# nrontsis/PILCO

Hardware: AMD Instinct MI355X
Metric: moment-matching rollouts/sec (N=1000,D=10,E=10,H=40) (higher is better)
Workload: dtype f64

## Files before the change

pilco_amd/csrc/prep_device.h:

```cpp
#pragma once
#include "glue_device.h"
#include "pair_device.h"

namespace pilco {

constexpr int PREP_TAB_DOUBLES = FEXP_TN + 8;
__host__ __device__ constexpr size_t prep_region_doubles(int DT) {
    const size_t stage = 256 * (size_t)(DT + 1),
                 ops = mm_kp(DT) <= 16 ? (size_t)mm_kp(DT) * (64 + 256) + 256 + (DT <= 14 ? 16 * 64 + 256 + 8 * 64 : 0) : 0;
    const size_t pair_blk = (size_t)4 * DT + 2 * (size_t)DT * DT + 4 + (stage > ops ? stage : ops);
    const size_t mean_blk = (size_t)2 * DT + 2 * (size_t)DT * DT + 4 + 9 * (size_t)(DT + 1) + 2 * (size_t)DT + 512 * (size_t)(DT + 2);
    return pair_blk > mean_blk ? pair_blk : mean_blk;
}

template <int DT>
__device__ __forceinline__ void prep_wt_constants(const MMModel& md, const MMWork& wk, int pl, double* sm) {
    const int R = wt_rows_per_pair(wk), t = threadIdx.x;
    if (wt_rows_dealt(wk) && t < R && pl * R + t < md.E * md.D) {
        const double l = md.ls[pl * R + t];
        sm[3 * DT + 2 * DT * DT + 4 + t] = 1.0 / (l * l);
    }
}

template <int DT, bool FUSED, int NTHR, bool PRE = false>
__device__ __forceinline__ void prep_mean_block(const MMModel& md, const MMWork& wk, int al, int chm, double* sm,
                                                const double* jm, const double* js,
                                                const double la_t, const double var_a) {
    const int D = md.D, npad = md.npad;
    const int t = threadIdx.x, lane = t & 63;
    const int w = __builtin_amdgcn_readfirstlane(t >> 6);
    const bool act = (NTHR == 512) || t < 512;
    const int a = al * wk.nranks + wk.rank;
    double* s_m = sm;
    double* s_ia = s_m + DT;
    double* s_s = s_ia + DT;
    double* s_T = s_s + DT * DT;
    double* s_sc = s_T + DT * DT;
    double* red = s_sc + 4;
    double* colbuf = red + 9 * (DT + 1);
    double* zst = colbuf + 2 * DT;
    double* bst = zst + 512 * (DT + 1);
    constexpr int LDZ = DT | 1;
    if constexpr (!PRE) {
        if (t < DT) {
            s_m[t] = (t < D) ? (FUSED ? jm[t] : wk.in_m[t]) : 0.0;
            s_ia[t] = (t < D) ? 1.0 / la_t : 0.0;
        }
        for (int e = t; e < D * D; e += 512) s_s[e] = FUSED ? js[e] : wk.in_s[e];
        for (int e = t; e < DT * DT; e += 512) s_T[e] = 0.0;
        __syncthreads();
    }
    const bool dbgm = (t == 0 && al == 0 && chm == 0);
    DBG_STAMP(wk, 40, dbgm);
    const int rpc = npad >> __builtin_ctz(wk.NCHM);
    const int i_begin = chm * rpc, i_end = i_begin + rpc;
    if (w == 0) {
        double col[DT];
        const int c = lane;
        const bool in_s = c < D;
        const double ic = in_s ? s_ia[c] : 0.0;
        double sv[DT], ir[DT];
#pragma unroll
        for (int r = 0; r < DT; ++r) {
            sv[r] = s_s[(in_s && r < D) ? r * D + c : 0];
            ir[r] = s_ia[r];
        }
#pragma unroll
        for (int r = 0; r < DT; ++r) {
            const double sval = (in_s && r < D) ? sv[r] : 0.0;
            col[r] = c < DT ? fma(sval, ir[r] * ic, (r == c) ? 1.0 : 0.0) : ((c < 2 * DT && c - DT == r) ? 1.0 : 0.0);
        }
        __builtin_amdgcn_s_setprio(3);
        const double detB = gj_wave<DT>(col, colbuf, lane);
        __builtin_amdgcn_s_setprio(0);
        if (c >= DT && c < DT + D) {
            const int cc = c - DT;
#pragma unroll
            for (int r = 0; r < DT; ++r)
                if (r < D) s_T[r * DT + cc] = col[r] * s_ia[r] * s_ia[cc];
        }
        if (lane == 0) s_sc[1] = var_a * fast_rsqrt(detB);
    } else if (act) {
        const int idx = (w - 1) * 64 + lane;
        constexpr int NB = (512 * DT + 447) / 448;
        double sv[NB], bv[2];
#pragma unroll
        for (int k = 0; k < NB; ++k) {
            const int e = idx + 448 * k, d = e >> 9, i = i_begin + (e & 511);
            sv[k] = (e < 512 * D && i < md.n && i < i_end) ? md.Pt[(long)d * npad + i] : 0.0;
        }
#pragma unroll
        for (int k = 0; k < 2; ++k) {
            const int r = idx + 448 * k;
            bv[k] = (r < 512 && i_begin + r < i_end) ? md.beta[mm_beta_row(md, a) * npad + i_begin + r] : 0.0;
        }
#pragma unroll
        for (int k = 0; k < NB; ++k) {
            const int e = idx + 448 * k, d = e >> 9, r = e & 511, i = i_begin + r;
            if (e < 512 * D) zst[r * LDZ + d] = (i < md.n && i < i_end) ? sv[k] - s_m[d] : 0.0;
        }
#pragma unroll
        for (int k = 0; k < 2; ++k)
            if (idx + 448 * k < 512) bst[idx + 448 * k] = bv[k];
    }
    __syncthreads();
    DBG_STAMP(wk, 41, dbgm);
    double g = 0.0;
    double h[DT];
#pragma unroll
    for (int d = 0; d < DT; ++d) h[d] = 0.0;
    for (int r0 = 0; r0 < rpc; r0 += 512) {
        if (r0 > 0) {
            __syncthreads();
            for (int e = t; act && e < 512 * D; e += 512) {
                const int d = e >> 9, r = e & 511;
                const int i = i_begin + r0 + r;
                zst[r * LDZ + d] = (i < md.n && i < i_end) ? md.Pt[(long)d * npad + i] - s_m[d] : 0.0;
            }
            if (act) bst[t] = (i_begin + r0 + t < i_end) ? md.beta[mm_beta_row(md, a) * npad + i_begin + r0 + t] : 0.0;
            __syncthreads();
        }
        if (act && i_begin + r0 + t < i_end) {
            double zeta[DT];
#pragma unroll
            for (int d = 0; d < DT; ++d) zeta[d] = (d < D) ? zst[t * LDZ + d] : 0.0;
            double hq = 0.0;
#pragma unroll
            for (int c = 0; c < DT; ++c) {
                double inner = 0.5 * s_T[c * DT + c] * zeta[c];
#pragma unroll
                for (int r = c + 1; r < DT; ++r) inner = fma(s_T[c * DT + r], zeta[r], inner);
                hq = fma(zeta[c], inner, hq);
            }
            const double lb = exp(-hq) * bst[t];
            g += lb;
#pragma unroll
            for (int d = 0; d < DT; ++d) h[d] = fma(zeta[d], lb, h[d]);
        }
    }
    DBG_STAMP(wk, 42, dbgm);
    double* hs = red + 8 * (DT + 1);
    __syncthreads();
    if (act) {
        zst[t] = g;
#pragma unroll
        for (int d = 0; d < DT; ++d)
            if (d < D) zst[(1 + d) * 512 + t] = h[d];
    }
    __syncthreads();
    for (int k = w; act && k < 1 + D; k += 8) {
        double acc = zst[k * 512 + lane];
#pragma unroll
        for (int j = 1; j < 8; ++j) acc += zst[k * 512 + 64 * j + lane];
        acc = wave_sum_lane63(acc);
        if (lane == 63) hs[k] = acc;
    }
    DBG_STAMP(wk, 43, dbgm);
    __syncthreads();
    if (t < 1 + D) {
        double v;
        if (t == 0) {
            v = s_sc[1] * hs[0];
        } else {
            double acc = 0.0;
            _Pragma("unroll 8") for (int k = 0; k < D; ++k) acc = fma(s_T[(t - 1) * DT + k], hs[1 + k], acc);
            v = s_sc[1] * acc;
        }
        store_wt(&wk.mean_part[((long)al * wk.NCHM + chm) * (1 + D) + t], v);
    }
    DBG_STAMP(wk, 44, dbgm);
}

template <int DT>
__device__ __forceinline__ void small_sweep(const MMModel& md, const MMWork& wk, int pl, int item, int i_begin, int c_begin, int ncols, const double* Al, const double* Bl,
                                            const double* vl, const double* Zl, double* bbl, double* csl, double* tail, bool act) {
    constexpr int KC = mm_kp(DT) / 4;
    constexpr bool VSEP = mm_vsep(DT);
    const int D = md.D, npad = md.npad, t = threadIdx.x, lane = t & 63, lr = lane >> 4, lc = lane & 15;
    const int w = __builtin_amdgcn_readfirstlane(t >> 6);
    const double* tab = tail;
    int a, b;
    local_pair_ab(wk, md.E, pl, a, b);
    const bool diag = (a == b);
    const double* beta_a = md.beta + mm_beta_row(md, a) * npad;
    const double* beta_b = md.beta + mm_beta_row(md, b) * npad;
    const double* iKa = (diag && md.iK) ? md.iK + mm_ik_blk(md, a) * npad * npad : nullptr;
    if (act)
        for (int e = t; e < 256; e += 512) bbl[e] = e < npad ? beta_b[e] : 0.0;
    for (int e = t; e < 8 * 64; e += 512) csl[e] = 0.0;
    __syncthreads();
    const int rg = w >> 2, cq = w & 3;
    const int i0l = 32 * rg, i0 = i_begin + i0l;
    const int cpw = ncols / 4, jb = c_begin + cpw * cq, je = jb + cpw;
    double rf[2][KC], brow[2];
#pragma unroll
    for (int rt = 0; rt < 2; ++rt) {
        brow[rt] = beta_a[i0 + 16 * rt + lc];
#pragma unroll
        for (int c = 0; c < KC; ++c) rf[rt][c] = Al[(4 * c + lr) * 64 + i0l + 16 * rt + lc];
    }
    const __amdgpu_buffer_rsrc_t rIK = buf_rsrc_uniform(iKa ? iKa : beta_a);
    unsigned ik_off[2][4];
#pragma unroll
    for (int r = 0; r < 4; ++r)
#pragma unroll
        for (int rt = 0; rt < 2; ++rt) ik_off[rt][r] = ((unsigned)(lr + 4 * r) * (unsigned)npad + (unsigned)(i0 + 16 * rt + lc)) * 8u;
    const int dsel = lc <= D ? lc : D;
    d4 acc[2] = {d4{0.0, 0.0, 0.0, 0.0}, d4{0.0, 0.0, 0.0, 0.0}};
    double* myslice = csl + w * 64;
    auto sweep = [&](auto mode_c) {
        constexpr int MODE = decltype(mode_c)::value;
        double ikv[4][2][4];
        if (MODE == 1) {
#pragma unroll
            for (int sidx = 0; sidx < 4; ++sidx) {
                const int j0 = jb + 16 * sidx;
#pragma unroll
                for (int rt = 0; rt < 2; ++rt)
#pragma unroll
                    for (int r = 0; r < 4; ++r)
                        ikv[sidx][rt][r] = (j0 < je && j0 >= i0) ? buf_ld(rIK, ik_off[rt][r], (unsigned)j0 * (unsigned)npad * 8u) : 0.0;
            }
        }
#pragma unroll
        for (int sidx = 0; sidx < 4; ++sidx) {
            const int j0 = jb + 16 * sidx;
            if (j0 >= je) break;
            if (MODE != 0 && j0 < i0) continue;
            double cf[KC], a2[4], bcol[4], vj[4];
#pragma unroll
            for (int c = 0; c < KC; ++c) cf[c] = Bl[(4 * c + lr) * 256 + j0 + lc];
#pragma unroll
            for (int r = 0; r < 4; ++r) {
                bcol[r] = bbl[j0 + lr + 4 * r];
                vj[r] = VSEP ? vl[j0 + lr + 4 * r] : 0.0;
                a2[r] = Bl[dsel * 256 + j0 + 4 * r + lr];
            }
            double csum[4] = {0.0, 0.0, 0.0, 0.0};
#pragma unroll
            for (int rt = 0; rt < 2; ++rt) {
                const int it = i0 + 16 * rt;
                const double om = j0 > it ? 2.0 : (j0 == it ? 1.0 : 0.0);
                d4 e = {0.0, 0.0, 0.0, 0.0};
#pragma unroll
                for (int c = 0; c < KC; ++c) {
                    e = __builtin_amdgcn_mfma_f64_16x16x4f64(cf[c], rf[rt][c], e, 0, 0, 0);
                    if (c == 0) MFMA_PIN(e, cf[0], rf[rt][0]);
                }
                MFMA_RESULT_FENCE(e);
                double wl[4];
#pragma unroll
                for (int r = 0; r < 4; ++r) {
                    const double l = fexp(VSEP ? e[r] + vj[r] : e[r], tab);
                    if (MODE == 0) {
                        wl[r] = bcol[r] * l;
                        csum[r] = fma(brow[rt], l, csum[r]);
                    } else {
                        double wgt = brow[rt] * bcol[r];
                        if (MODE == 1) wgt -= ikv[sidx][rt][r];
                        wl[r] = (wgt * om) * l;
                        csum[r] += wl[r];
                    }
                }
#pragma unroll
                for (int r = 0; r < 4; ++r) {
                    acc[rt] = __builtin_amdgcn_mfma_f64_16x16x4f64(wl[r], a2[r], acc[rt], 0, 0, 0);
                    MFMA_PIN(acc[rt], wl[r], a2[r]);
                }
            }
#pragma unroll
            for (int r = 0; r < 4; ++r) {
                double v = csum[r];
                v = dpp_add<0x111, 0xf>(v);
                v = dpp_add<0x112, 0xf>(v);
                v = dpp_add<0x114, 0xf>(v);
                v = dpp_add<0x118, 0xf>(v);
                if (lc == 15) myslice[j0 - jb + lr + 4 * r] = v;
            }
        }
    };
    if (act) {
        if (!diag) sweep(std::integral_constant<int, 0>{});
        else if (iKa) sweep(std::integral_constant<int, 1>{});
        else sweep(std::integral_constant<int, 2>{});
    }
    d4 G = {0.0, 0.0, 0.0, 0.0}, Gc = {0.0, 0.0, 0.0, 0.0};
    const int rlane = (lane & 48) | (D & 15);
    if (act) {
#pragma unroll
        for (int rt = 0; rt < 2; ++rt)
#pragma unroll
            for (int r = 0; r < 4; ++r) {
                const int il = i0l + 16 * rt + 4 * r + lr, i = i_begin + il;
                const bool valid = i < md.n;
                const double zt = (valid && lc <= D) ? Zl[lc * 64 + il] : 0.0;
                const double bs = !valid ? 0.0 : (diag ? 1.0 : beta_a[i]);
                const double ri = __shfl(acc[rt][r], rlane);
                const double x = acc[rt][r];
                const double mp = bs == 0.0 ? 0.0 : (lc < D ? fma(0.5 * ri, zt, x) : x);
                const double za = zt * bs;
                G = __builtin_amdgcn_mfma_f64_16x16x4f64(za, mp, G, 0, 0, 0);
                MFMA_PIN(G, za, mp);
            }
    }
    __syncthreads();
    if (act) {
        const int cw8 = ncols / 8;
#pragma unroll
        for (int k = 0; k < 8; ++k) {
            if (4 * k >= cw8) break;
            const int jl = cw8 * w + 4 * k + lr, j = c_begin + jl;
            const int q = jl / cpw;
            double cj = 0.0, wt = 0.0;
            if (j < md.n) {
                const int jj = jl - cpw * q;
                cj = (csl[q * 64 + jj] + csl[(4 + q) * 64 + jj]) * (diag ? 1.0 : bbl[j]);
                wt = lc <= D ? Bl[lc * 256 + j] : 0.0;
            }
            const double ca = cj * wt;
            Gc = __builtin_amdgcn_mfma_f64_16x16x4f64(ca, wt, Gc, 0, 0, 0);
            MFMA_PIN(Gc, ca, wt);
        }
    }
    __syncthreads();
    double* red = const_cast<double*>(Bl);
    double* gout = wk.sw_gpart + ((long)pl * wk.NT + item) * 512;
    const int tN = ((D & 15) >> 2) * 64 + (D & 3) * 16 + (D & 15);
    for (int blk = 0; blk < 2; ++blk) {
        if (blk) __syncthreads();
        d4 v4 = blk ? Gc : G;
        MFMA_RESULT_FENCE(v4);
        if (act) {
#pragma unroll
            for (int r = 0; r < 4; ++r) red[w * 256 + r * 64 + lane] = v4[r];
        }
        __syncthreads();
        if (t < 256) {
            double v = red[t];
#pragma unroll
            for (int k = 1; k < 8; ++k) v += red[k * 256 + t];
            gout[blk * 256 + t] = v;
            if (blk == 0 && t == tN) {
                double* o = wk.pair_part + ((long)pl * wk.NT + item) * 2;
                store_wt(o, v);
                store_wt(o + 1, 0.0);
            }
        }
    }
}

template <int DT, bool FUSED, int NTHR, bool FPAIR = false, bool PRE = false>
__device__ __forceinline__ void prep_work(const MMModel& md, const MMWork& wk, const PrepReward& pr, const GlueArgs& g, const GlueLds& L,
                                          double* sm_all, int glue_doubles, int bx, int by, int gx, int gy, int pair_a, int pair_b, double pre_la, double pre_lb,
                                          double pre_var) {
    double* sm = sm_all + (FUSED ? glue_doubles : 0);
    const bool state_in = FUSED && (g.flags & GF_RBF_PRE);
    const double* jm = sm_all + (state_in ? 0 : L.o_js - L.nm);
    const double* js = sm_all + (state_in ? L.o_sx : L.o_js);
    if (bx >= wk.PL) {
        const int idx = (bx - wk.PL) * gy + by;
        const int nmean = wk.EL * wk.NCHM;
        const int slot = 64 + 2 * (by * gx + bx);
        if (wk.dbg && threadIdx.x == 0 && slot < 958) wk.dbg[slot] = wall_clock64();
        if (idx < nmean) {
            prep_mean_block<DT, FUSED, NTHR, PRE>(md, wk, idx >> __builtin_ctz(wk.NCHM), idx & (wk.NCHM - 1), sm, jm, js, pre_la, pre_var);
            if (wk.dbg && threadIdx.x == 0 && slot < 958) wk.dbg[slot + 1] = wall_clock64();
            return;
        }
        if (idx != nmean || pr.n <= 0) return;
        const int E = pr.E, t = threadIdx.x;
        double* mx = sm;
        double* sx = mx + E;
        double* ws = sx + E * E;
        if (FUSED) {
            if (t < E) mx[t] = L.mx[t];
            for (int e = t; e < E * E; e += blockDim.x) sx[e] = L.sx[e];
        } else {
            if (t < E) mx[t] = pr.m_x[t];
            for (int e = t; e < E * E; e += blockDim.x) sx[e] = pr.s_x[e];
        }
        __syncthreads();
        double mu, var;
        reward_eval(pr.n, pr.rw, E, mx, sx, ws, false, mu, var);
        if (t == 0) pr.reward[0] += mu;
        if (wk.dbg && t == 0 && slot < 958) wk.dbg[slot + 1] = wall_clock64();
        return;
    }
    const int D = md.D, npad = md.npad;
    double* s_m = sm;
    double* s_ia2 = s_m + DT;
    double* s_ib2 = s_ia2 + DT;
    double* s_s = s_ib2 + DT;
    double* s_Q = s_s + DT * DT;
    double* s_sc = s_Q + DT * DT;
    double* colbuf = s_sc + 4;
    double* zst = colbuf + DT;
    const int t = threadIdx.x, lane = t & 63;
    const int w = __builtin_amdgcn_readfirstlane(t >> 6);
    const bool act = (NTHR == 512) || t < 512;
    const int grp = t >> 8, tl = t & 255;
    const int pl = bx, ch = by & (wk.NCH - 1), cs = by >> __builtin_ctz(wk.NCH);
    const bool dbg0 = (t == 0 && pl == 0 && ch == 0);
    DBG_STAMP(wk, 0, dbg0);
    if (wk.dbg && t == 0) wk.dbg[64 + 2 * (by * gx + bx)] = wall_clock64();
    if constexpr (!PRE) {
        if (t < DT) {
            double la = 1.0, lb = 1.0, mm = 0.0;
            if (t < D) {
                mm = FUSED ? jm[t] : wk.in_m[t];
                la = pre_la;
                lb = pre_lb;
            }
            s_m[t] = mm;
            s_ia2[t] = (t < D) ? 1.0 / (la * la) : 0.0;
            s_ib2[t] = (t < D) ? 1.0 / (lb * lb) : 0.0;
        }
        prep_wt_constants<DT>(md, wk, pl, sm);
        for (int e = t; e < D * D; e += 512) s_s[e] = FUSED ? js[e] : wk.in_s[e];
        for (int e = t; e < DT * DT; e += 512) s_Q[e] = 0.0;
        __syncthreads();
    }
    DBG_STAMP(wk, 1, dbg0);
    const int rpc = npad >> __builtin_ctz(wk.NCH);
    const int i_begin = ch * rpc, i_end = i_begin + rpc;
    const int side = grp;
    constexpr int LDZ = DT | 1;
    const bool fpair = FPAIR && wk.fuse_pair;
    const bool fplds = fpair && mm_kp(DT) <= 16 && rpc == 64;
    const int ncsg = (fplds && wk.NCS > 1) ? wk.NCS : 1, ncols = npad >> __builtin_ctz(ncsg), c_begin = cs * ncols, c_end = c_begin + ncols;
    double* Al = zst;
    double* Bl = Al + mm_kp(DT) * 64;
    double* vl = Bl + mm_kp(DT) * 256;
    const bool fsweep = fplds && DT <= 14 && wk.fuse_pair == 2;
    double* Zl = vl + 256;
    double* bbl = Zl + 16 * 64;
    double* csl = bbl + 256;
    const int st_begin = fpair ? 0 : i_begin, st_end = fpair ? npad : i_end;
    if (w != 0 && act) {
        const int idx = (w - 1) * 64 + lane;
        for (int e = idx; e < 256 * D; e += 448) {
            const int d = e >> 8, r = e & 255;
            const int i = st_begin + r;
            zst[r * LDZ + d] = (i < md.n && i < st_end) ? md.Pt[(long)d * npad + i] - s_m[d] : 0.0;
        }
        DBG_STAMP(wk, 7, t == 64 && pl == 0 && ch == 0);
    }
    const double logvar = pre_var;
    if (MM_ABL(wk, 2)) {
        if (t == 0) s_sc[0] = 1.0;
    } else if (w == 0) {
        double col[DT];
        const int c = lane;
        const int cc = c < DT ? c : c - DT;
        const bool in_s = cc < D && c < 2 * DT;
        const double lam = (c < DT && c < D) ? s_ia2[c] + s_ib2[c] : 0.0;
        double sv[DT];
#pragma unroll
        for (int r = 0; r < DT; ++r) sv[r] = s_s[(in_s && r < D) ? r * D + cc : 0];
#pragma unroll
        for (int r = 0; r < DT; ++r) {
            const double sval = (in_s && r < D) ? sv[r] : 0.0;
            col[r] = c < DT ? fma(sval, lam, (r == c) ? 1.0 : 0.0) : sval;
        }
        DBG_STAMP(wk, 5, dbg0);
        __builtin_amdgcn_s_setprio(3);
        const double det = gj_wave<DT>(col, colbuf, lane);
        __builtin_amdgcn_s_setprio(0);
        DBG_STAMP(wk, 6, dbg0);
        if (c >= DT && c < DT + D) {
#pragma unroll
            for (int r = 0; r < DT; ++r)
                if (r < D) s_Q[r * DT + (c - DT)] = 0.5 * col[r];
        }
        if (lane == 0) {
            s_sc[0] = fast_rsqrt(det);
            if (by == 0) store_wt(&wk.pair_isdet[pl], s_sc[0]);
        }
    }
    __syncthreads();
    DBG_STAMP(wk, 2, dbg0);
    const int KP = wk.KP;
    const int pa_ = pair_a, pb_ = pair_b;
    double* At = wk.At + (long)pl * KP * npad;
    double* Wb = wk.Wt + (long)pair_col_block(wk, pl, pb_) * KP * npad;
    double* vrow = wk.vcol + (long)pl * npad;
    const bool wt_dealt = wt_rows_dealt(wk);
    const bool wt_writer = !wt_dealt && pair_writes_wt(wk, md.E, pa_, pb_);
    const int wt_R = wt_rows_per_pair(wk);
    auto row = [&](const int i, const bool valid, const double (&zeta)[DT]) {
        const double* il2 = side ? s_ib2 : s_ia2;
        double x[DT], y[DT];
        double kk = logvar;
#pragma unroll
        for (int d = 0; d < DT; ++d) {
            x[d] = zeta[d] * il2[d];
            kk = fma(-0.5 * zeta[d], x[d], kk);
            y[d] = 0.0;
        }
        DBG_STAMP_ROW(wk, 34, dbg0);
#pragma unroll
        for (int c = 0; c < DT; ++c) {
            double qrow[DT];
#pragma unroll
            for (int r = 0; r < DT; ++r) qrow[r] = s_Q[c * DT + r];
#pragma unroll
            for (int r = 0; r < DT; ++r) y[r] = fma(qrow[r], x[c], y[r]);
            if ((c & 1) == 1) __builtin_amdgcn_sched_barrier(0);
        }
        double quad = 0.0;
#pragma unroll
        for (int r = 0; r < DT; ++r) quad = fma(x[r], y[r], quad);
        DBG_STAMP_ROW(wk, 35, dbg0);
        const double uv = valid ? (kk + quad) : 0.0;
        const double one = valid ? 1.0 : 0.0;
        if (fplds) {
            if (side == 0) {
                const int il = i - i_begin;
#pragma unroll
                for (int r = 0; r < DT; ++r)
                    if (r < D) Al[r * 64 + il] = 2.0 * y[r];
                Al[D * 64 + il] = uv;
                if (!wk.vsep) Al[(D + 1) * 64 + il] = one;
                for (int k = D + 2; k < KP; ++k) Al[k * 64 + il] = 0.0;
                if (fsweep) {
#pragma unroll
                    for (int r = 0; r < DT; ++r)
                        if (r < D) Zl[r * 64 + il] = x[r];
                    Zl[D * 64 + il] = one;
                }
            } else {
#pragma unroll
                for (int r = 0; r < DT; ++r)
                    if (r < D) Bl[r * 256 + i] = x[r];
                Bl[D * 256 + i] = one;
                if (wk.vsep) vl[i] = uv;
                else Bl[(D + 1) * 256 + i] = uv;
                for (int k = D + 2; k < KP; ++k) Bl[k * 256 + i] = 0.0;
            }
        } else if (side == 0) {
#pragma unroll
            for (int r = 0; r < DT; ++r)
                if (r < D) store_wt(&At[(long)r * npad + i], 2.0 * y[r]);
            store_wt(&At[(long)D * npad + i], uv);
        } else {
            if (wt_writer) {
#pragma unroll
                for (int r = 0; r < DT; ++r)
                    if (r < D) store_wt(&Wb[(long)r * npad + i], x[r]);
            }
            store_wt(&vrow[i], uv);
            if (wt_dealt) {
                for (int q = 0; q < wt_R; ++q) {
                    const int rr = pl * wt_R + q;
                    if (rr >= md.E * D) break;
                    int dd;
                    const int bb = idiv_s(rr, D, dd);
                    store_wt(&wk.Wt[((long)bb * KP + dd) * npad + i], zst[(i - st_begin) * LDZ + dd] * colbuf[q]);
                }
            }
        }
    };
    if (fplds) {
        const int r_begin = side ? c_begin : i_begin, r_end = side ? c_end : i_end;
        const bool has = act && r_begin + tl < r_end;
        const int i = r_begin + tl;
        double zeta[DT];
#pragma unroll
        for (int d = 0; d < DT; ++d) zeta[d] = (has && d < D) ? zst[(i - st_begin) * LDZ + d] : 0.0;
        __syncthreads();
        if (has) row(i, i < md.n, zeta);
    } else if (!MM_ABL(wk, 4) && act) {
        const int r_begin = (fpair && side) ? 0 : i_begin, r_end = (fpair && side) ? npad : i_end;
        if (r_begin + tl < r_end) {
            const int i = r_begin + tl;
            double zeta[DT];
#pragma unroll
            for (int d = 0; d < DT; ++d) zeta[d] = (d < D) ? zst[(i - st_begin) * LDZ + d] : 0.0;
            row(i, i < md.n, zeta);
        }
        for (int i = i_begin + tl + 256; i < i_end; i += 256) {
            const bool valid = i < md.n;
            double zeta[DT];
#pragma unroll
            for (int d = 0; d < DT; ++d) zeta[d] = (d < D && valid) ? md.Pt[(long)d * npad + i] - s_m[d] : 0.0;
            row(i, valid, zeta);
        }
    }
    DBG_STAMP(wk, 3, dbg0);
    if (fsweep) {
        small_sweep<DT>(md, wk, pl, by, i_begin, c_begin, ncols, Al, Bl, vl, Zl, bbl, csl, sm + prep_region_doubles(DT), act);
    } else if (fpair) {
        constexpr int KCP = mm_kp(DT) / 4;
        constexpr bool VSP = mm_vsep(DT);
        const double* tab = sm + prep_region_doubles(DT);
        double* wred = sm + prep_region_doubles(DT) + FEXP_TN;
        __syncthreads();
        int a, b;
        local_pair_ab(wk, md.E, pl, a, b);
        const bool diag = (a == b) && (md.iK != nullptr);
        const int nrg = rpc / (16 * PAIR_RT), ncs = max(1, 8 / nrg);
        double val = 0.0;
        if (act && w < nrg * ncs) {
            const int rg = w / ncs, cq = w - rg * ncs, ct = ncols / 16;
            const int i0 = i_begin + 16 * PAIR_RT * rg, jb = c_begin + 16 * (ct * cq / ncs), je = c_begin + 16 * (ct * (cq + 1) / ncs);
            const double* beta_a = md.beta + mm_beta_row(md, a) * npad;
            const double* beta_b = md.beta + mm_beta_row(md, b) * npad;
            const double* iKa = diag ? md.iK + mm_ik_blk(md, a) * npad * npad : nullptr;
            const PairOps po = pair_ops(wk, D, npad, pl, pair_col_block(wk, pl, b));
            if (fplds && mm_kp(DT) <= 16) {
                if (diag) val = pair_wave<KCP, true, VSP, true, true>(po, Al, Bl, vl, beta_a, beta_b, iKa, tab, npad, i0, jb, je, lane, 64, 256, i0 - i_begin);
                else val = pair_wave<KCP, false, VSP, true, true>(po, Al, Bl, vl, beta_a, beta_b, nullptr, tab, npad, i0, jb, je, lane, 64, 256, i0 - i_begin);
            } else if (diag) {
                val = pair_wave<KCP, true, VSP, true>(po, nullptr, nullptr, nullptr, beta_a, beta_b, iKa, tab, npad, i0, jb, je, lane);
            } else {
                val = pair_wave<KCP, false, VSP, true>(po, nullptr, nullptr, nullptr, beta_a, beta_b, nullptr, tab, npad, i0, jb, je, lane);
            }
            for (int off = 32; off > 0; off >>= 1) val += __shfl_down(val, off);
        }
        if (act && lane == 0) wred[w] = val;
        __syncthreads();
        if (t == 0) {
            double* out = wk.pair_part + ((long)pl * wk.NT + by) * 2;
            store_wt(out, ((wred[0] + wred[1]) + (wred[2] + wred[3])) + ((wred[4] + wred[5]) + (wred[6] + wred[7])));
            store_wt(out + 1, 0.0);
        }
    }
    DBG_STAMP(wk, 4, dbg0);
    if (wk.dbg && t == 0) wk.dbg[65 + 2 * (by * gx + bx)] = wall_clock64();
}

}
```

Measured before the change: 416.4.

## Compute per-row quadratic forms with f64 MFMA tiles instead of scalar rows

Measured after the change: 416.9 (median of 6 runs). About the same (+0.1%).

```diff
diff --git a/pilco_amd/csrc/prep_device.h b/pilco_amd/csrc/prep_device.h
--- a/pilco_amd/csrc/prep_device.h
+++ b/pilco_amd/csrc/prep_device.h
@@ -570,20 +570,119 @@
         __syncthreads();
         if (has) row(i, i < md.n, zeta);
     } else if (!MM_ABL(wk, 4) && act) {
+        constexpr int KC = (DT + 3) / 4, MT = (DT + 15) / 16;
+        const int lr = lane >> 4, lc = lane & 15, ws = tl >> 6;
+        const double* il2 = side ? s_ib2 : s_ia2;
+        double qa[MT][KC], il[KC];
+#pragma unroll
+        for (int c = 0; c < KC; ++c) {
+            const int k = 4 * c + lr;
+            il[c] = k < DT ? il2[k] : 0.0;
+#pragma unroll
+            for (int mt = 0; mt < MT; ++mt) qa[mt][c] = (k < DT && 16 * mt + lc < DT) ? s_Q[(16 * mt + lc) * DT + k] : 0.0;
+        }
+        constexpr int TG = DT <= 16 ? 4 : 1;
+        auto tiles = [&](const int (&i)[TG], const bool (&in_r)[TG], const double (&zeta)[TG][KC]) {
+            double x[TG][KC], part[TG];
+            d4 y[TG][MT];
+#pragma unroll
+            for (int g = 0; g < TG; ++g) {
+                part[g] = 0.0;
+#pragma unroll
+                for (int c = 0; c < KC; ++c) {
+                    x[g][c] = zeta[g][c] * il[c];
+                    part[g] = fma(-0.5 * zeta[g][c], x[g][c], part[g]);
+                }
+            }
+#pragma unroll
+            for (int g = 0; g < TG; ++g)
+#pragma unroll
+                for (int mt = 0; mt < MT; ++mt) {
+                    y[g][mt] = d4{0.0, 0.0, 0.0, 0.0};
+#pragma unroll
+                    for (int c = 0; c < KC; ++c) {
+                        y[g][mt] = __builtin_amdgcn_mfma_f64_16x16x4f64(qa[mt][c], x[g][c], y[g][mt], 0, 0, 0);
+                        if (c == 0) MFMA_PIN(y[g][mt], qa[mt][0], x[g][0]);
+                    }
+                }
+#pragma unroll
+            for (int g = 0; g < TG; ++g)
+#pragma unroll
+                for (int mt = 0; mt < MT; ++mt) {
+                    MFMA_RESULT_FENCE(y[g][mt]);
+#pragma unroll
+                    for (int r = 0; r < 4; ++r)
+                        if (4 * mt + r < KC) part[g] = fma(x[g][4 * mt + r], y[g][mt][r], part[g]);
+                }
+#pragma unroll
+            for (int g = 0; g < TG; ++g) part[g] += __shfl_xor(part[g], 16);
+#pragma unroll
+            for (int g = 0; g < TG; ++g) part[g] += __shfl_xor(part[g], 32);
+#pragma unroll
+            for (int g = 0; g < TG; ++g) {
+                if (!in_r[g]) continue;
+                const double uv = i[g] < md.n ? logvar + part[g] : 0.0;
+                if (side == 0) {
+#pragma unroll
+                    for (int mt = 0; mt < MT; ++mt)
+#pragma unroll
+                        for (int r = 0; r < 4; ++r) {
+                            const int m = 16 * mt + lr + 4 * r;
+                            if (m < D) store_wt(&At[(long)m * npad + i[g]], 2.0 * y[g][mt][r]);
+                        }
+                    if (lr == 0) store_wt(&At[(long)D * npad + i[g]], uv);
+                } else {
+                    if (wt_writer) {
+#pragma unroll
+                        for (int c = 0; c < KC; ++c)
+                            if (4 * c + lr < D) store_wt(&Wb[(long)(4 * c + lr) * npad + i[g]], x[g][c]);
+                    }
+                    if (lr == 0) store_wt(&vrow[i[g]], uv);
+                    if (wt_dealt) {
+                        for (int q = lr; q < wt_R; q += 4) {
+                            const int rr = pl * wt_R + q;
+                            if (rr >= md.E * D) break;
+                            int dd;
+                            const int bb = idiv_s(rr, D, dd);
+                            store_wt(&wk.Wt[((long)bb * KP + dd) * npad + i[g]], zst[(i[g] - st_begin) * LDZ + dd] * colbuf[q]);
+                        }
+                    }
+                }
+            }
+        };
         const int r_begin = (fpair && side) ? 0 : i_begin, r_end = (fpair && side) ? npad : i_end;
-        if (r_begin + tl < r_end) {
-            const int i = r_begin + tl;
-            double zeta[DT];
-#pragma unroll
-            for (int d = 0; d < DT; ++d) zeta[d] = (d < D) ? zst[(i - st_begin) * LDZ + d] : 0.0;
-            row(i, i < md.n, zeta);
-        }
-        for (int i = i_begin + tl + 256; i < i_end; i += 256) {
-            const bool valid = i < md.n;
-            double zeta[DT];
-#pragma unroll
-            for (int d = 0; d < DT; ++d) zeta[d] = (d < D && valid) ? md.Pt[(long)d * npad + i] - s_m[d] : 0.0;
-            row(i, valid, zeta);
+#pragma unroll
+        for (int k0 = 0; k0 < 4; k0 += TG) {
+            if (r_begin + 64 * ws + 16 * k0 >= r_end) break;
+            int i[TG];
+            bool in_r[TG];
+            double zeta[TG][KC];
+#pragma unroll
+            for (int g = 0; g < TG; ++g) {
+                i[g] = r_begin + 64 * ws + 16 * (k0 + g) + lc;
+                in_r[g] = i[g] < r_end;
+#pragma unroll
+                for (int c = 0; c < KC; ++c) zeta[g][c] = (in_r[g] && 4 * c + lr < D) ? zst[(i[g] - st_begin) * LDZ + 4 * c + lr] : 0.0;
+            }
+            tiles(i, in_r, zeta);
+        }
+        for (int i0 = i_begin + 256 + 64 * ws; i0 < i_end; i0 += 256) {
+#pragma unroll
+            for (int k0 = 0; k0 < 4; k0 += TG) {
+                if (i0 + 16 * k0 >= i_end) break;
+                int i[TG];
+                bool in_r[TG];
+                double zeta[TG][KC];
+#pragma unroll
+                for (int g = 0; g < TG; ++g) {
+                    i[g] = i0 + 16 * (k0 + g) + lc;
+                    in_r[g] = i[g] < i_end;
+                    const bool valid = in_r[g] && i[g] < md.n;
+#pragma unroll
+                    for (int c = 0; c < KC; ++c) zeta[g][c] = (valid && 4 * c + lr < D) ? md.Pt[(long)(4 * c + lr) * npad + i[g]] - s_m[4 * c + lr] : 0.0;
+                }
+                tiles(i, in_r, zeta);
+            }
         }
     }
     DBG_STAMP(wk, 3, dbg0);
```
